# alibaba/pairec

Measured on AMD Instinct MI355X. Metric: ranked items/sec, 5k-cand DNN rank (recall top-5000 of 100M x 128 -> DNN3 -> fuse -> sort), higher is better.
Workload: dtype bf16x3; 1 GPU; configs[1]+[2]: recall 5k of 100000000x128 fp32 table in HBM -> 3-layer DNN rank (256-512-256-1, bf16 MFMA with split hi + lo operands = bf16x3, fp32-accurate scores) -> RankScore fusion (fp64) -> ItemRankScore sort; candidates_per_request=5000, table_rows=100000000, dim=128, table_dist=uniform, batches_in_flight=2, contexts=2, all_batches_on_predicted_thresholds=True, batches_re_run_after_a_failed_plan=0, parallelism=1 GPU

## Files before the change

### pairec_amd/csrc/recall.hip

```cpp
#include "common.hpp"
#include "bitonic_reg.hpp"
#include "split_sort.hpp"

#include <type_traits>

namespace pg {

typedef float f32x16 __attribute__((ext_vector_type(16)));
typedef float f32x4 __attribute__((ext_vector_type(4)));

constexpr int kPieceRows = 32;
constexpr int kPieceCols = 32;
constexpr int kPieceBytes = kPieceRows * kPieceCols * 4;
constexpr int kPieceDmas = kPieceBytes / 1024;
constexpr int kPieceQuads = kPieceCols / 4;
constexpr int kRingSlots = 4;
constexpr int kScanWaves = 8;
constexpr int kScanLdsRing = kScanWaves * kRingSlots * kPieceBytes;
constexpr int kStageCap = 280;
constexpr int kStageBytes = kStageCap * 12 + 512;
constexpr int kScanLds = kScanLdsRing + kScanWaves * kStageBytes;

__device__ __forceinline__ uint32_t f32_ordered_bits(float f) {
    const uint32_t b = __float_as_uint(f);
// ... 260 lines not shown
                    __builtin_amdgcn_s_waitcnt(0x0F70);
                } else {
#pragma unroll
                    for (int r = 0; r < 16; ++r) {
                        const bool p = (pass >> r) & 1u;
                        const uint64_t m = __builtin_amdgcn_ballot_w64(p);
                        if (m != 0) {
                            if (p) {
                                const uint32_t pos = st_n + __builtin_amdgcn_mbcnt_hi((uint32_t)(m >> 32),
                                                         __builtin_amdgcn_mbcnt_lo((uint32_t)m, 0u));
                                const uint32_t row = row0 + (r & 3) + 8 * (r >> 2) + 4 * h;
                                st_key[pos] = topk_key(acc[c][r], row);
                                st_q[pos] = qid;
                            }
                            st_n += __popcll(m);
                        }
                    }
                }
            }
        }
    }
    flush();
    wait_vmcnt<0>();
}

typedef __bf16 bf16x8 __attribute__((ext_vector_type(8)));
typedef float f32x8 __attribute__((ext_vector_type(8)));

constexpr int kScreenMaxNQB = 8;
constexpr int kScreenLds = 163840;
constexpr float kScreenEps = 0.008f;

struct ScreenArgs {
    const void* tab16;
    const uint4* qb16;
    const float* thr_screen;
    uint32_t* susp_cnt;
    uint32_t* susp;
    uint32_t* overflow;
    uint32_t cap, nq, rb_begin, rb_end, row_end, stride, perm_mul, perm_mod;
    const float* blk_norm2;
    const float* eps_unit;
    char* rec;
    uint32_t* rec_cnt;
    uint32_t rec_cap;
    char* rec_pool;
    uint32_t rec_pool_cap, rec_waves;
    uint32_t early_share;
    const float* blk_nxmin;
    const float* l2_b;
    const float* nx_rows;
};

constexpr uint32_t kRecBytes = 80;
constexpr uint32_t kRecOvfWord = 1 + kMaxQueries + 1;

template <int DIM, int NQB, int WAVES, int SPLIT = 1, int VAR = 0, bool I8 = false, int QH = 1, int L2 = 0>
__global__ __launch_bounds__(64 * WAVES, WAVES / 4) void screen_kernel(ScreenArgs a) {
    static_assert(SPLIT == 1 && VAR == 0);
    static_assert(!L2 || (I8 && QH == 1), "squared-Euclidean screen: the int8 kernels of <= 128 queries");
    extern __shared__ __attribute__((aligned(16))) char smem[];
    constexpr int EB = I8 ? 1 : 2;
    constexpr int kCols16 = 128 / EB;
    static_assert(DIM % kCols16 == 0, "a shadow row is a whole number of 128-B lines");
    constexpr int PPB = DIM / kCols16;
    constexpr int NS = kScanLdsRing / (WAVES * kPieceBytes);
    constexpr int ND = kPieceDmas;
    constexpr int KS = DIM * EB / 32;
    typedef int i32x16 __attribute__((ext_vector_type(16)));
    typedef int i32x4 __attribute__((ext_vector_type(4)));
    using AccT = typename std::conditional<I8, i32x16, f32x16>::type;
    using ThrT = typename std::conditional<I8, int, float>::type;
    constexpr int kBLds = QH > 1 ? 2048 : 0;
    constexpr int kStageBytesW = (kScreenLds - kScanLdsRing - kBLds) / WAVES;
    constexpr int NQT = NQB * QH;
    static_assert(QH == 1 || PPB == 1, "query halves: one piece per block");
    constexpr int kCap = (kStageBytesW - NQT * 256 - 16) / 8;
    constexpr int kScanWaves = WAVES;
    const int lane = threadIdx.x & 63;
    const int wave = __builtin_amdgcn_readfirstlane(threadIdx.x >> 6);
    const uint32_t gw = blockIdx.x * kScanWaves + wave;
    const uint32_t W = gridDim.x * kScanWaves;
    const int i32 = lane & 31;
    const int h = lane >> 5;

    uint4 bfrag[NQT][KS];
    ThrT thr_s[NQT];
    float eu[NQT];
    float la[NQT];
    bool active[NQT];
    char* const b_lds = smem + kScreenLds - kBLds;
    if constexpr (QH > 1) {
        if (wave == 0) {
            *reinterpret_cast<uint4*>(b_lds + lane * 16) = a.qb16[((NQT - 1) * KS + KS - 2) * 64 + lane];
            *reinterpret_cast<uint4*>(b_lds + 1024 + lane * 16) = a.qb16[((NQT - 1) * KS + KS - 1) * 64 + lane];
        }
        __syncthreads();
    }
#pragma unroll
    for (int c = 0; c < NQT; ++c) {
#pragma unroll
        for (int ks = 0; ks < KS; ++ks) {
            if (QH > 1 && c == NQT - 1 && ks >= KS - 2) bfrag[c][ks] = make_uint4(0, 0, 0, 0);
            else bfrag[c][ks] = a.qb16[(c * KS + ks) * 64 + lane];
        }
        active[c] = (uint32_t)(c * 32 + i32) < a.nq;
        if constexpr (I8) thr_s[c] = active[c] ? __float_as_int(a.thr_screen[c * 32 + i32]) : 0x7fffffff;
        else thr_s[c] = active[c] ? a.thr_screen[c * 32 + i32] : __builtin_inff();
        eu[c] = (!I8 && active[c]) ? a.eps_unit[c * 32 + i32] : 0.0f;
        if constexpr (L2 != 0) {
            la[c] = active[c] ? a.thr_screen[c * 32 + i32] : __builtin_inff();
            eu[c] = active[c] ? a.l2_b[c * 32 + i32] : 0.0f;
        }
    }
#pragma unroll
    for (int c = 0; c < NQT; ++c) {
#pragma unroll
        for (int ks = 0; ks < KS; ++ks) {
            if (QH > 1 && c == NQT - 1 && ks >= KS - 2) continue;
            if (NQT > 4)
                asm volatile("" : "+a"(bfrag[c][ks].x), "+a"(bfrag[c][ks].y), "+a"(bfrag[c][ks].z), "+a"(bfrag[c][ks].w));
            else
                asm volatile("" : "+v"(bfrag[c][ks].x), "+v"(bfrag[c][ks].y), "+v"(bfrag[c][ks].z), "+v"(bfrag[c][ks].w));
        }
        asm volatile("" : "+v"(thr_s[c]));
        if (!I8 || L2) asm volatile("" : "+v"(eu[c]));
        if (L2) asm volatile("" : "+v"(la[c]));
    }

    uint32_t voff[ND];
#pragma unroll
    for (int n = 0; n < ND; ++n) {
        const int S = n * 64 + lane;
        const int i = S >> 3, p = S & 7;
        voff[n] = (uint32_t)(i * DIM * EB + 16 * ((p + (i >> 1)) & 7));
    }
    const uint32_t lds_wave_u = __builtin_amdgcn_readfirstlane(
        (uint32_t)(uintptr_t)((__attribute__((address_space(3))) char*)smem) + wave * (NS * kPieceBytes));
    char* const lds_ptr = smem + wave * (NS * kPieceBytes);
    const int rd_row = i32 * 128;
    const int rd_rot = (i32 >> 1) * 16;

    const uint32_t total = a.rb_end - a.rb_begin;
    uint32_t first, nblk;
    if (WAVES == 8 && a.early_share != 512) {
        const uint32_t P = gridDim.x * 4;
        const uint32_t pb = (total + P - 1) / P;
        const uint32_t pbase = (blockIdx.x * 4 + (wave & 3)) * pb;
        const uint32_t pend = pbase + pb < total ? pbase + pb : total;
        uint32_t cut = pbase + (uint32_t)(((uint64_t)pb * a.early_share + 512) >> 10);
        if (cut > pend) cut = pend;
        first = wave < 4 ? pbase : cut;
        const uint32_t last = wave < 4 ? cut : pend;
        nblk = first < last ? last - first : 0;
    } else {
        const uint32_t bpw = (total + W - 1) / W;
        first = gw * bpw;
        nblk = first < total ? (total - first < bpw ? total - first : bpw) : 0;
    }
    if (nblk == 0) {
        if (QH > 1 && lane == 0) a.rec_cnt[gw] = 0;
        return;
    }

    constexpr int D = (PPB - 1 + NS - 1) / PPB;
    const bool strided = a.stride != 1;
    const uint32_t L0 = a.rb_begin + first;
    uint32_t walk_slot = strided ? (uint32_t)(((uint64_t)L0 * a.perm_mul) % a.perm_mod) : L0;
    uint32_t walk_n = 0;
    auto next_phys = [&]() -> uint32_t {
        const uint32_t ph = strided ? slot_block(walk_slot, a.stride) : walk_slot;
        if (walk_n + 1 < nblk) {
            ++walk_n;
            if (strided) {
                walk_slot += a.perm_mul;
                if (walk_slot >= a.perm_mod) walk_slot -= a.perm_mod;
            } else {
                ++walk_slot;
            }
        }
        return __builtin_amdgcn_readfirstlane(ph);
    };
    uint32_t phys[D + 1];
#pragma unroll
    for (int j = 0; j <= D; ++j) phys[j] = next_phys();
    auto piece_addr = [&](int rel_piece, uint32_t t, const char*& ub, uint32_t& dst) {
        const uint32_t ph = phys[rel_piece / PPB];
        const char* base = (const char*)a.tab16 + (uint64_t)ph * (uint64_t)(kPieceRows * DIM * EB) + (rel_piece % PPB) * 128;
// ... 2 lines not shown
        ub = (const char*)(((uint64_t)hi << 32) | lo);
        dst = lds_wave_u + __builtin_amdgcn_readfirstlane(t % NS) * kPieceBytes;
    };

    uint32_t* const st_row = reinterpret_cast<uint32_t*>(smem + kScanLdsRing + wave * kStageBytesW);
    uint32_t* const st_q = st_row + kCap;
    uint32_t* const st_cnt = st_q + kCap;
    uint32_t* const st_base = st_cnt + NQT * 32;
    uint32_t st_n = 0;
    auto flush = [&]() {
#pragma unroll
        for (int part = 0; part < (NQT + 1) / 2; ++part)
            if (lane + 64 * part < NQT * 32) st_cnt[lane + 64 * part] = 0;
        for (uint32_t e0 = 0; e0 < st_n; e0 += 64) {
            const uint32_t e = e0 + lane;
            if (e < st_n) atomicAdd(&st_cnt[st_q[e]], 1u);
        }
#pragma unroll
        for (int part = 0; part < (NQT + 1) / 2; ++part) {
            const int q = lane + 64 * part;
            if (q < NQT * 32) {
                const uint32_t c = st_cnt[q];
                st_base[q] = c ? atomicAdd(&a.susp_cnt[q], c) : 0u;
                st_cnt[q] = 0;
            }
        }
        for (uint32_t e0 = 0; e0 < st_n; e0 += 64) {
            const uint32_t e = e0 + lane;
            if (e < st_n) {
                const uint32_t q = st_q[e];
                const uint32_t pos = st_base[q] + atomicAdd(&st_cnt[q], 1u);
                if (pos < a.cap) a.susp[(uint64_t)q * a.cap + pos] = st_row[e];
                else *a.overflow = 1u;
            }
        }
        st_n = 0;
        __builtin_amdgcn_s_waitcnt(0x0F70);
    };

#pragma unroll
    for (int t = 0; t < NS - 1; ++t) {
        const char* src;
        uint32_t dst;
        piece_addr(t, t, src, dst);
#pragma unroll
        for (int n = 0; n < ND; ++n) dma_one(src, dst + n * 1024, voff[n], 0.0f);
    }

    if constexpr (QH > 1) {
        constexpr uint32_t kRecStage = (uint32_t)kStageBytesW / kRecBytes;
        char* const rec_lds = smem + kScanLdsRing + wave * kStageBytesW;
        char* const rec_glb = a.rec + (size_t)gw * a.rec_cap * kRecBytes;
        uint32_t rec_st = 0, rec_total = 0;
        auto rec_flush = [&]() {
            if (rec_total + rec_st > a.rec_cap) {
                uint32_t g = 0;
                if (lane == 0) g = atomicAdd(&a.rec_cnt[a.rec_waves], rec_st);
                g = __builtin_amdgcn_readfirstlane(g);
                if (g + rec_st > a.rec_pool_cap) {
                    if (lane == 0) { *a.overflow = 1u; a.overflow[kRecOvfWord] = 1u; }
                } else {
                    char* const dst = a.rec_pool + (size_t)g * kRecBytes;
                    for (uint32_t o = lane * 16; o < rec_st * kRecBytes; o += 1024)
                        *reinterpret_cast<i32x4*>(dst + o) = *reinterpret_cast<const i32x4*>(rec_lds + o);
                }
            } else {
                char* const dst = rec_glb + (size_t)rec_total * kRecBytes;
                for (uint32_t o = lane * 16; o < rec_st * kRecBytes; o += 1024)
                    *reinterpret_cast<i32x4*>(dst + o) = *reinterpret_cast<const i32x4*>(rec_lds + o);
                rec_total += rec_st;
            }
            rec_st = 0;
        };
        for (uint32_t b = 0; b < nblk; ++b) {
            wait_vmcnt<ND * (NS - 2)>();
            const char* nb_src;
            uint32_t nb_dst;
            piece_addr(NS - 1, b + NS - 1, nb_src, nb_dst);
            const char* slot = lds_ptr + (b % NS) * kPieceBytes + rd_row;
            f32x4 q4[4];
#pragma unroll
            for (int j = 0; j < 4; ++j) q4[j] = *reinterpret_cast<const f32x4*>(slot + (((2 * j + h) * 16 - rd_rot) & 112));
            __builtin_amdgcn_sched_barrier(0);
#pragma unroll
            for (int n = 0; n < ND; ++n)
                dma_one(nb_src, nb_dst + n * 1024, voff[n], q4[n].x);
            const uint32_t cur_phys = phys[0];
#pragma unroll
            for (int j = 0; j < D; ++j) phys[j] = phys[j + 1];
            phys[D] = next_phys();
            const uint32_t row0 = cur_phys * kPieceRows;
#pragma unroll
            for (int half = 0; half < QH; ++half) {
                AccT acc[NQB];
#pragma unroll
                for (int c = 0; c < NQB; ++c)
#pragma unroll
                    for (int r = 0; r < 16; ++r) acc[c][r] = 0;
#pragma unroll
                for (int ksl = 0; ksl < 4; ++ksl)
#pragma unroll
                    for (int c = 0; c < NQB; ++c) {
                        uint4 bq;
                        if (half * NQB + c == NQT - 1 && ksl >= KS - 2) bq = *reinterpret_cast<const uint4*>(b_lds + (ksl - (KS - 2)) * 1024 + lane * 16);
                        else bq = bfrag[half * NQB + c][ksl];
                        acc[c] = __builtin_amdgcn_mfma_i32_32x32x32_i8(__builtin_bit_cast(i32x4, q4[ksl]),
                                                                       __builtin_bit_cast(i32x4, bq), acc[c], 0, 0, 0);
                    }
                uint64_t cmask[NQB];
                bool hit[NQB];
                uint64_t any_mask = 0;
#pragma unroll
                for (int c = 0; c < NQB; ++c) {
                    int m = acc[c][0];
#pragma unroll
                    for (int r = 1; r < 16; ++r) m = acc[c][r] > m ? acc[c][r] : m;
                    hit[c] = m >= thr_s[half * NQB + c];
                    cmask[c] = __builtin_amdgcn_ballot_w64(hit[c]);
                    any_mask |= cmask[c];
                }
                if (any_mask != 0) {
#pragma unroll
                    for (int c = 0; c < NQB; ++c) {
                        if (cmask[c] == 0) continue;
                        uint64_t pend = cmask[c];
                        bool mine = hit[c];
                        for (;;) {
                            const uint32_t n = (uint32_t)__popcll(pend);
                            if (rec_st + n > kRecStage && rec_st != 0) rec_flush();
                            const uint32_t pre = __builtin_amdgcn_mbcnt_hi((uint32_t)(pend >> 32),
                                                                           __builtin_amdgcn_mbcnt_lo((uint32_t)pend, 0u));
                            const bool take = mine && pre < kRecStage;
                            if (take) {
                                char* const r = rec_lds + (rec_st + pre) * kRecBytes;
#pragma unroll
                                for (int jj = 0; jj < 4; ++jj) {
                                    const i32x4 v = {acc[c][4 * jj], acc[c][4 * jj + 1], acc[c][4 * jj + 2], acc[c][4 * jj + 3]};
                                    *reinterpret_cast<i32x4*>(r + 16 * jj) = v;
                                }
                                *reinterpret_cast<uint2*>(r + 64) = make_uint2(row0, (uint32_t)((half * NQB + c) * 32 + i32) | ((uint32_t)h << 8));
                            }
                            rec_st += n < kRecStage ? n : kRecStage;
                            if (n <= kRecStage) break;
                            mine = mine && !take;
                            pend = __builtin_amdgcn_ballot_w64(mine);
                        }
                    }
                }
            }
        }
        rec_flush();
        if (lane == 0) a.rec_cnt[gw] = rec_total;
    } else {
    for (uint32_t b = 0; b < nblk; ++b) {
        AccT acc[NQB];
#pragma unroll
        for (int c = 0; c < NQB; ++c)
#pragma unroll
            for (int r = 0; r < 16; ++r) acc[c][r] = 0;
#pragma unroll
        for (int pc = 0; pc < PPB; ++pc) {
            const uint32_t t = b * PPB + pc;
            wait_vmcnt<ND * (NS - 2)>();
            const char* nb_src;
            uint32_t nb_dst;
            piece_addr(pc + NS - 1, t + NS - 1, nb_src, nb_dst);
            const char* slot = lds_ptr + (t % NS) * kPieceBytes + rd_row;
            f32x4 q4[4];
#pragma unroll
            for (int j = 0; j < 4; ++j) {
                const int quad = 2 * j + h;
                q4[j] = *reinterpret_cast<const f32x4*>(slot + ((quad * 16 - rd_rot) & 112));
            }
            __builtin_amdgcn_sched_barrier(0);
#pragma unroll
            for (int n = 0; n < ND; ++n)
                dma_one(nb_src, nb_dst + n * 1024, voff[n], q4[n].x);
#pragma unroll
            for (int ksl = 0; ksl < 4; ++ksl) {
                const bf16x8 af = __builtin_bit_cast(bf16x8, q4[ksl]);
                const int ks = pc * 4 + ksl;
#pragma unroll
                for (int c = 0; c < NQB; ++c) {
                    if constexpr (I8)
                        acc[c] = __builtin_amdgcn_mfma_i32_32x32x32_i8(__builtin_bit_cast(i32x4, q4[ksl]),
                                                                       __builtin_bit_cast(i32x4, bfrag[c][ks]), acc[c], 0, 0, 0);
                    else
                        acc[c] = __builtin_amdgcn_mfma_f32_32x32x16_bf16(af, __builtin_bit_cast(bf16x8, bfrag[c][ks]), acc[c], 0, 0, 0);
                }
            }
        }
        const uint32_t cur_phys = phys[0];
#pragma unroll
// ... 53 lines not shown
            any_mask |= cmask[c];
        }
        if (any_mask != 0) {
            const uint32_t row0 = cur_phys * kPieceRows;
#pragma unroll
            for (int c = 0; c < NQB; ++c) {
                if (cmask[c] == 0) continue;
                uint32_t m16 = 0;
#pragma unroll
                for (int r = 0; r < 16; ++r) {
                    if constexpr (L2 == 2) {
                        const float g = __fmaf_rn((float)acc[c][r], eu[c], -nxr[r]);
                        asm volatile("v_cmp_nlt_f32 vcc, %1, %2\n\tv_addc_co_u32 %0, vcc, %0, %0, vcc"
                                     : "+v"(m16) : "v"(g), "v"(la[c]) : "vcc");
                    } else if constexpr (I8)
                        asm volatile("v_cmp_ge_i32 vcc, %1, %2\n\tv_addc_co_u32 %0, vcc, %0, %0, vcc"
                                     : "+v"(m16) : "v"(acc[c][r]), "v"(cut[c]) : "vcc");
                    else
                        asm volatile("v_cmp_nlt_f32 vcc, %1, %2\n\tv_addc_co_u32 %0, vcc, %0, %0, vcc"
                                     : "+v"(m16) : "v"(acc[c][r]), "v"(cut[c]) : "vcc");
                }
                if (row0 + kPieceRows > a.row_end) {
#pragma unroll
                    for (int r = 0; r < 16; ++r)
                        if (row0 + (r & 3) + 8 * (r >> 2) + 4 * h >= a.row_end) m16 &= ~(1u << (15 - r));
                }
                for (;;) {
                    const bool p = m16 != 0;
                    const uint64_t bm = __builtin_amdgcn_ballot_w64(p);
                    if (bm == 0) break;
                    const uint32_t n = __popcll(bm);
                    if (st_n + n > (uint32_t)kCap) flush();
                    if (p) {
                        const int r = 15 - __builtin_ctz(m16);
                        const uint32_t pos = st_n + __builtin_amdgcn_mbcnt_hi((uint32_t)(bm >> 32),
                                                 __builtin_amdgcn_mbcnt_lo((uint32_t)bm, 0u));
                        st_row[pos] = row0 + (r & 3) + 8 * (r >> 2) + 4 * h;
                        st_q[pos] = (uint32_t)(c * 32 + i32);
                        m16 &= m16 - 1;
                    }
                    st_n += n;
                }
            }
        }
    }
    }
    if constexpr (QH == 1) flush();
    wait_vmcnt<0>();
}

__device__ __forceinline__ uint32_t rec_mask(const char* r, const float* __restrict__ thr_screen, uint32_t row_end, uint32_t& q,
                                             uint32_t& row0h) {
    typedef int i32x4 __attribute__((ext_vector_type(4)));
    const uint2 tag = *reinterpret_cast<const uint2*>(r + 64);
    q = tag.y & 255u;
    const uint32_t h = (tag.y >> 8) & 1u;
    row0h = tag.x + 4 * h;
    const int t = __float_as_int(thr_screen[q]);
    uint32_t m = 0;
#pragma unroll
    for (int jj = 0; jj < 4; ++jj) {
        const i32x4 v = *reinterpret_cast<const i32x4*>(r + 16 * jj);
#pragma unroll
        for (int e = 0; e < 4; ++e) {
            const int rr = 4 * jj + e;
            if (v[e] >= t && row0h + (rr & 3) + 8 * (rr >> 2) < row_end) m |= 1u << rr;
        }
    }
    return m;
}
constexpr uint32_t kRecPoolSlice = 8192;
__global__ __launch_bounds__(1024) void screen_decode_kernel(const char* __restrict__ rec, const uint32_t* __restrict__ rec_cnt,
                                                             uint32_t rec_cap, uint32_t rec_waves, const char* __restrict__ rec_pool,
                                                             uint32_t rec_pool_cap, const float* __restrict__ thr_screen, uint32_t row_end,
                                                             uint32_t* __restrict__ susp_cnt, uint32_t* __restrict__ susp,
                                                             uint32_t cap, uint32_t* __restrict__ overflow) {
    __shared__ uint32_t cntq[kMaxQueries], baseq[kMaxQueries], nreg[8];
    constexpr uint32_t kKeep = 12288;
    __shared__ uint2 keep[kKeep];
    const bool pool = blockIdx.x >= rec_waves / 8;
    if (threadIdx.x < kMaxQueries) cntq[threadIdx.x] = 0;
    if (threadIdx.x < 8) {
        uint32_t n;
        if (pool) {
            const uint32_t filled = rec_cnt[rec_waves] < rec_pool_cap ? rec_cnt[rec_waves] : rec_pool_cap;
            const uint32_t begin = (blockIdx.x - rec_waves / 8) * kRecPoolSlice;
            n = threadIdx.x == 0 && begin < filled ? (filled - begin < kRecPoolSlice ? filled - begin : kRecPoolSlice) : 0u;
        } else {
            const uint32_t n_raw = rec_cnt[blockIdx.x * 8 + threadIdx.x];
            n = n_raw < rec_cap ? n_raw : rec_cap;
        }
        nreg[threadIdx.x] = n;
    }
    __syncthreads();
    for (int pass = 0; pass < 2; ++pass) {
        uint32_t off = 0;
        for (uint32_t w = 0; w < 8; ++w) {
            const uint32_t n = nreg[w];
            const char* const base = pool ? rec_pool + (size_t)(blockIdx.x - rec_waves / 8) * kRecPoolSlice * kRecBytes
                                          : rec + (size_t)(blockIdx.x * 8 + w) * rec_cap * kRecBytes;
            for (uint32_t e = threadIdx.x; e < n; e += 1024) {
                uint32_t q, row0h, m;
                const uint32_t slot = off + e;
                if (pass == 1 && slot < kKeep) {
                    const uint2 kp = keep[slot];
                    row0h = kp.x;
                    q = kp.y & 0xffffu;
                    m = kp.y >> 16;
                } else {
                    m = rec_mask(base + (size_t)e * kRecBytes, thr_screen, row_end, q, row0h);
                    if (pass == 0 && slot < kKeep) keep[slot] = make_uint2(row0h, q | (m << 16));
                }
                if (m == 0) continue;
                const uint32_t nh = __popc(m);
                if (pass == 0) {
                    atomicAdd(&cntq[q], nh);
                } else {
                    uint32_t pos = baseq[q] + atomicAdd(&cntq[q], nh);
                    if (pos + nh > cap) { *overflow = 1u; continue; }
                    while (m) {
                        const uint32_t rr = __builtin_ctz(m);
                        m &= m - 1;
                        susp[(uint64_t)q * cap + pos++] = row0h + (rr & 3) + 8 * (rr >> 2);
                    }
                }
            }
            off += n;
        }
        __syncthreads();
        if (pass == 0 && threadIdx.x < kMaxQueries) {
            const uint32_t c = cntq[threadIdx.x];
            baseq[threadIdx.x] = c ? atomicAdd(&susp_cnt[threadIdx.x], c) : 0u;
            cntq[threadIdx.x] = 0;
        }
        __syncthreads();
    }
}

template <int DIM>
__device__ __forceinline__ void rescore_gather(f32x4 (&buf)[16], const float* __restrict__ tab, uint32_t row, int ph, int lane) {
#pragma unroll
    for (int i = 0; i < 16; ++i) {
        const uint32_t r_i = (uint32_t)__shfl((int)row, 4 * i + (lane >> 4), 64);
        buf[i] = reinterpret_cast<const f32x4*>(tab + (size_t)r_i * DIM + ph * 64)[lane & 15];
    }
}
template <int ROWB>
__device__ __forceinline__ void rescore_walk(const f32x4 (&buf)[16], char* my, const float* qs, int ph, int lane, float& s) {
#pragma unroll
    for (int i = 0; i < 16; ++i)
        *reinterpret_cast<f32x4*>(my + (4 * i + (lane >> 4)) * ROWB + (lane & 15) * 16) = buf[i];
    __builtin_amdgcn_fence(__ATOMIC_RELEASE, "wavefront");
    __builtin_amdgcn_wave_barrier();
#pragma unroll
    for (int k = 0; k < 16; ++k) {
        const float4 x = *reinterpret_cast<const float4*>(my + lane * ROWB + k * 16);
        const float4 y = *reinterpret_cast<const float4*>(&qs[ph * 64 + 4 * k]);
        s = __fmaf_rn(x.x, y.x, s);
        s = __fmaf_rn(x.y, y.y, s);
        s = __fmaf_rn(x.z, y.z, s);
        s = __fmaf_rn(x.w, y.w, s);
        if ((k & 3) == 3) __builtin_amdgcn_sched_barrier(0);
    }
    __builtin_amdgcn_wave_barrier();
}

template <int DIM, bool L2 = false>
__global__ __launch_bounds__(256) void rescore_kernel(const float* __restrict__ tab, const float* __restrict__ qpad,
                                                      const float* __restrict__ thr,
                                                      const uint32_t* __restrict__ susp,
                                                      const uint32_t* __restrict__ susp_cnt, uint32_t cap,
                                                      uint32_t* __restrict__ cnt, uint64_t* __restrict__ cand,
                                                      uint32_t* __restrict__ overflow, uint32_t scap, uint32_t n_rows,
                                                      const float* __restrict__ nx = nullptr, const float* __restrict__ nqv = nullptr,
                                                      RowFilter filter = RowFilter()) {
    constexpr int kRowB = 64 * 4 + 16;
// ... 69 lines not shown
        uint32_t pos = base_s + before;
        for (int j = 0; j < w; ++j) pos += wsum[j];
        if (keep) {
            if (pos < cap) cand[(uint64_t)q * cap + pos] = topk_key(s, row);
            else *overflow = 1u;
        }
        __syncthreads();
        row = row_next;
    }
    if (n_raw > scap && threadIdx.x == 0) *overflow = 1u;
}

__global__ void screen_prep_kernel(const float* __restrict__ qpad, uint32_t dim,
                                   uint4* __restrict__ qb16, float* __restrict__ eps) {
    const uint32_t KS = dim / 16;
    const uint32_t i = blockIdx.x * blockDim.x + threadIdx.x;
    if (i < (uint32_t)kScreenMaxNQB * KS * 64) {
        const uint32_t lane = i & 63, ks = (i >> 6) % KS, c = (i >> 6) / KS;
        const float* q = qpad + (size_t)(c * 32 + (lane & 31)) * dim + ks * 16 + 8 * (lane >> 5);
        uint32_t w[4];
        for (int e = 0; e < 4; ++e) {
            auto rne = [](float x) -> uint32_t {
                uint32_t b = __float_as_uint(x);
                if ((b & 0x7FFFFFFFu) > 0x7F800000u) return (b >> 16) | 0x40u;
                b += 0x7FFFu + ((b >> 16) & 1u);
                return b >> 16;
            };
            w[e] = rne(q[2 * e]) | (rne(q[2 * e + 1]) << 16);
        }
        qb16[i] = make_uint4(w[0], w[1], w[2], w[3]);
    }
    if (i < (uint32_t)kMaxQueries) {
        double ss = 0.0;
        for (uint32_t k = 0; k < dim; ++k) {
            const double v = (double)qpad[(size_t)i * dim + k];
            ss += v * v;
        }
        eps[i] = (float)(sqrt(ss) * (double)kScreenEps * 1.0001) + 1e-30f;
    }
}

__global__ void screen_thr_kernel(const float* __restrict__ thr, const float* __restrict__ eps, float max_norm,
                                  float* __restrict__ thr_screen) {
    const uint32_t q = threadIdx.x;
    if (q >= (uint32_t)kMaxQueries) return;
    const float t = thr[q], e = eps[q];
    float v = t;
    if (!(e == e) || e > 1e28f || !(t == t) || !(e * max_norm < 1e35f)) v = -__builtin_inff();
    thr_screen[q] = v;
}

__global__ __launch_bounds__(128) void screen_prep8_kernel(const float* __restrict__ qpad, uint32_t dim,
                                                            float max_norm, float resid, uint4* __restrict__ qb8,
                                                            float* __restrict__ eps, float* __restrict__ qscale) {
    __shared__ float sq[32];
    const uint32_t tid = threadIdx.x, c = blockIdx.x;
    {
        const uint32_t ql = tid >> 2, qi = c * 32 + ql, part = tid & 3, per = dim / 4;
        const float* q = qpad + (size_t)qi * dim + part * per;
        float mx = 0.0f;
        bool bad = false;
        for (uint32_t k = 0; k < per; ++k) {
            const float v = fabsf(q[k]);
            if (!(v <= 3.0e38f)) bad = true;
            mx = fmaxf(mx, v);
        }
        mx = fmaxf(mx, __shfl_xor(mx, 1, 64));
        mx = fmaxf(mx, __shfl_xor(mx, 2, 64));
        bad = (__shfl_xor((int)bad, 1, 64) | (int)bad) != 0;
        bad = (__shfl_xor((int)bad, 2, 64) | (int)bad) != 0;
        const float sc = fmaxf(mx / 127.0f, 1e-30f);
        double ss = 0.0, dd = 0.0;
        for (uint32_t k = 0; k < per; ++k) {
            const double v = (double)q[k];
            int Q = __float2int_rn(q[k] / sc);
            Q = Q > 127 ? 127 : (Q < -127 ? -127 : Q);
            const double d = v - (double)sc * (double)Q;
            ss += v * v;
            dd += d * d;
        }
        ss += __shfl_xor(ss, 1, 64);
        ss += __shfl_xor(ss, 2, 64);
        dd += __shfl_xor(dd, 1, 64);
        dd += __shfl_xor(dd, 2, 64);
        if (part == 0) {
            const double nq = sqrt(ss), dq = sqrt(dd);
            const double e = ((double)resid * nq + ((double)max_norm + (double)resid) * dq) * 1.0001 +
                             1e-5 * (double)max_norm * nq + 1e-30;
            eps[qi] = bad ? __builtin_nanf("") : (float)(e * 1.000001);
            qscale[qi] = sc;
            sq[ql] = sc;
        }
    }
    __syncthreads();
    const uint32_t KS = dim / 32;
    for (uint32_t i = tid; i < KS * 64; i += blockDim.x) {
        const uint32_t lane = i & 63, ks = i >> 6;
        const uint32_t ql = lane & 31;
        const float* q = qpad + (size_t)(c * 32 + ql) * dim + ks * 32 + 16 * (lane >> 5);
        const float sc = sq[ql];
        uint32_t w[4];
        for (int e = 0; e < 4; ++e) {
            uint32_t word = 0;
            for (int b = 0; b < 4; ++b) {
                int Q = __float2int_rn(q[4 * e + b] / sc);
                Q = Q > 127 ? 127 : (Q < -127 ? -127 : Q);
                word |= (uint32_t)(Q & 0xff) << (8 * b);
            }
            w[e] = word;
        }
        qb8[(c * KS + ks) * 64 + lane] = make_uint4(w[0], w[1], w[2], w[3]);
    }
}

__global__ void screen_thr8_kernel(const float* __restrict__ thr, const float* __restrict__ eps,
                                   const float* __restrict__ qscale, float s_x, float* __restrict__ thr_screen) {
    const uint32_t q = threadIdx.x;
    if (q >= (uint32_t)kMaxQueries) return;
    const float t = thr[q], e = eps[q];
    int T = (int)0x80000000;
    if (e == e && e <= 1e30f && t == t && t > -__builtin_inff()) {
        const double v = floor(((double)t - (double)e) / ((double)s_x * (double)qscale[q])) - 1.0;
        T = v >= 2147483647.0 ? 0x7fffffff : (v <= -2147483648.0 ? (int)0x80000000 : (int)v);
    }
    thr_screen[q] = __int_as_float(T);
}

__global__ void screen_thr8_l2_kernel(const float* __restrict__ thr, const float* __restrict__ eps, const float* __restrict__ qscale,
                                      const float* __restrict__ nqv, float s_x, float max_norm, float* __restrict__ a_out,
                                      float* __restrict__ b_out, int per_row) {
    const uint32_t q = threadIdx.x;
    if (q >= (uint32_t)kMaxQueries) return;
    const float t = thr[q], e = eps[q];
    const double nq = (double)nqv[q], N = (double)max_norm;
    const double sq = (double)s_x * (double)qscale[q];
    float A = -__builtin_inff(), B = 0.0f;
    if (e == e && e <= 1e30f && t == t && t > -__builtin_inff() && sq > 0.0 && nq == nq && nq < 1e30) {
        const double delta = 2e-6 * (N * N + nq + 2.0 * N * sqrt(nq)) + 1e-30;
        if (per_row) {
            const double c = (double)t - 2.0 * delta + nq - 2.0 * (double)e;
            A = (float)(c - fabs(c) * 1e-6 - 1e-30);
            B = (float)(2.0 * sq);
            if (!(A == A) || !(B == B) || B > 1e30f) { A = -__builtin_inff(); B = 0.0f; }
        } else {
            const double a = (((double)t - delta + nq) * 0.5 - (double)e) / sq;
            const double b = 0.5 / sq;
            A = (float)(a - fabs(a) * 1e-6 - 1.0);
            B = (float)(b * (1.0 - 1e-6));
            if (!(A == A) || !(B == B) || B > 1e30f) { A = -__builtin_inff(); B = 0.0f; }
        }
    }
    a_out[q] = A;
    b_out[q] = B;
}
__global__ void block_nxmin_kernel(const float* __restrict__ nx, uint64_t rows, float* __restrict__ out, uint32_t nblocks,
                                   double* __restrict__ stats) {
    const uint32_t b = blockIdx.x * blockDim.x + threadIdx.x;
    double slack = 0.0, sum = 0.0;
    if (b < nblocks) {
        float m = __builtin_inff();
        for (uint32_t i = 0; i < (uint32_t)kPieceRows; ++i) {
            const uint64_t r = (uint64_t)b * kPieceRows + i;
            if (r < rows) m = fminf(m, nx[r]);
        }
// ... 1282 lines not shown
    bool last_was_i4m = false;
    bool last_was_r2 = false;
    bool exact_chunks = false;

    explicit PlanRun(RecallJob* job) : j(job), ctx(job->ctx), t(job->t), rs(job->rs) {}

    int scan_range(uint32_t rb, uint32_t cb, uint32_t st, bool thr_is_open, bool allow_i4 = false) {
        std::vector<hipEvent_t>& pool = *j->events;
        while (pool.size() < 2 * (size_t)(n_ev + 1)) {
            hipEvent_t e;
            PG_HIP(hipEventCreate(&e));
            pool.push_back(e);
        }
        if (j->timers) PG_HIP(hipEventRecord(pool[2 * n_ev], ctx->stream));
        const uint32_t nq = j->nq;
        if (j->screen && !thr_is_open && !exact_chunks) {
            ScreenArgs sa;
            sa.tab16 = t->shadow_is_i8 ? (const void*)t->d8 : (const void*)t->d16;
            sa.blk_norm2 = t->dnorm2;
            sa.eps_unit = rs.eps;
            sa.qb16 = rs.qb16;
            sa.thr_screen = rs.thr_screen;
            sa.susp_cnt = rs.susp_cnt;
            sa.susp = rs.susp;
            sa.overflow = rs.overflow;
            sa.cap = rs.cap;
            sa.nq = nq;
            sa.rb_begin = rb;
            sa.rb_end = rb + cb;
            sa.row_end = j->rows;
            sa.stride = st;
            sa.perm_mul = j->perm_mul;
            sa.perm_mod = j->sample_blocks;
            int rc2;
            const bool records = t->shadow_is_i8 && nq > 128;
            sa.rec = nullptr;
            sa.rec_cnt = nullptr;
            sa.rec_cap = 0;
            sa.rec_pool = nullptr;
            sa.rec_pool_cap = sa.rec_waves = 0;
            sa.early_share = records ? ctx->knobs.screen_early_share : ctx->knobs.screen_early_share_narrow;
            sa.blk_nxmin = j->l2 && !j->l2_per_row ? t->d_nxmin : nullptr;
            sa.nx_rows = j->l2 && j->l2_per_row ? t->d_nx : nullptr;
            sa.l2_b = j->l2 ? rs.thr_ref : nullptr;
            const uint32_t rec_waves = (uint32_t)ctx->num_cus * 8u;
            if (records) {
                const uint64_t rsc = t->rec_scale ? t->rec_scale : 1;
                uint32_t cap_w = (uint32_t)(((uint64_t)kMaxQueries * j->k * 4 * rsc / rec_waves + 255) / 256 * 256);
                const uint32_t pairs = (uint32_t)ctx->num_cus * 4u;
                const uint32_t pb = (kCandSlack / 2 / kPieceRows + pairs - 1) / pairs;
                const uint32_t es = sa.early_share > 512 ? sa.early_share : 1024 - sa.early_share;
                uint32_t eb = (uint32_t)(((uint64_t)pb * es + 512) >> 10) + 1;
                if (eb > pb) eb = pb;
                const uint32_t floor_w = eb * 512;
                if (cap_w < floor_w) cap_w = floor_w;
                const uint32_t pool_cap = (uint32_t)(((uint64_t)kMaxQueries * j->k * 2 * rsc + kRecPoolSlice - 1) / kRecPoolSlice * kRecPoolSlice);
                if ((rc2 = scratch_carve(ctx, kSlotHitRecords, [&](Carve& c) {
                        sa.rec_cnt = c.take<uint32_t>((size_t)rec_waves + 1);
                        sa.rec = (char*)c.bytes(((size_t)rec_waves * cap_w + pool_cap) * kRecBytes);
                    }))) return rc2;
                sa.rec_cap = cap_w;
                sa.rec_pool = sa.rec + (size_t)rec_waves * cap_w * kRecBytes;
                sa.rec_pool_cap = pool_cap;
                sa.rec_waves = rec_waves;
                PG_HIP(hipMemsetAsync(sa.rec_cnt, 0, (size_t)(rec_waves + 1) * 4, ctx->stream));
            }
            if (!susp_clean) PG_HIP(hipMemsetAsync(rs.susp_cnt, 0, sizeof(uint32_t) * kMaxQueries, ctx->stream));
            susp_clean = false;
            last_full_screened = true;
            last_was_r2 = false;
            const bool i4 = j->screen4 && allow_i4 && st == 1 && (rb & 1) == 0 && (((rb + cb) & 1) == 0 || rb + cb == j->nblocks);
            const bool i4m = j->screen4m && allow_i4 && st == 1 && (rb & 1) == 0 && (((rb + cb) & 1) == 0 || rb + cb == j->nblocks);
            const uint32_t scap = i4 ? rs.cap * (uint32_t)(kMaxQueries / kI4MaxQueries) : rs.cap;
            const uint64_t r_begin = (uint64_t)rb * kPieceRows;
            const uint64_t r_end = (uint64_t)(rb + cb) * kPieceRows < j->rows ? (uint64_t)(rb + cb) * kPieceRows : j->rows;
            if (i4) {
                if ((rc2 = screen4_launch(ctx, t, rs, nq, (uint32_t)r_begin, (uint32_t)r_end, scap, j->l2 ? rs.pred_ms : nullptr))) return rc2;
                j->scan_bytes += (r_end - r_begin) * (j->l2 ? 72 : 68);
            } else if (i4m) {
                if ((rc2 = screen4m_launch(ctx, t, rs, nq, (uint32_t)r_begin, (uint32_t)r_end, rs.cap * (uint32_t)(kMaxQueries / kI4mMaxQueries), susp2_clean))) return rc2;
                susp2_clean = false;
                j->scan_bytes += (r_end - r_begin) * 68;
                last_was_i4m = true;
            } else {
                last_was_i4m = false;
                if ((rc2 = dispatch_screen(ctx, t->dim, t->shadow_is_i8, sa))) return rc2;
                if (records) {
                    screen_decode_kernel<<<rec_waves / 8 + sa.rec_pool_cap / kRecPoolSlice, 1024, 0, ctx->stream>>>(
                        sa.rec, sa.rec_cnt, sa.rec_cap, rec_waves, sa.rec_pool, sa.rec_pool_cap, rs.thr_screen, j->rows,
                                                                            rs.susp_cnt, rs.susp, rs.cap, rs.overflow);
                    PG_HIP(hipGetLastError());
                }
                j->scan_bytes += (uint64_t)cb * kPieceRows * t->dim * (t->shadow_is_i8 ? 1 : 2);
            }
            j->scanned_rows += (uint64_t)cb * kPieceRows;
            const dim3 rg(i4 ? screen4_rescore_blocks() : kRescoreBlocksPerQuery, nq);
            const bool r2 = j->stage2 && t->shadow_is_i8 && !i4 && !i4m && !j->l2 && t->dim == 128;
            if (r2) {
                if ((rc2 = rescreen16_launch(ctx, t, rs, nq))) return rc2;
                last_was_r2 = true;
                rescore_kernel<128><<<rg, 256, 0, ctx->stream>>>(t->d, rs.qpad, rs.thr, rs.susp2, rs.susp2w_cnt, rs.cap,
                                                                 rs.cnt, rs.cand[cur], rs.overflow, rs.cap, j->rows, nullptr, nullptr, j->filter);
            } else if (j->l2)
                rescore_kernel<128, true><<<rg, 256, 0, ctx->stream>>>(t->d, rs.qpad, rs.thr, rs.susp, rs.susp_cnt, rs.cap, rs.cnt,
                                                                       rs.cand[cur], rs.overflow, scap, j->rows, t->d_nx, rs.pred_ms, j->filter);
            else if (t->dim == 64)
                rescore_kernel<64><<<rg, 256, 0, ctx->stream>>>(t->d, rs.qpad, rs.thr, rs.susp, rs.susp_cnt, rs.cap,
// ... 61 lines not shown
    }
    int grow_scan(uint32_t nb, uint32_t st, uint32_t kk, double growth, bool safe) {
        uint32_t rb = 0;
        while (rb < nb) {
            uint32_t chunk_rows;
            if (rb == 0) {
                chunk_rows = next_pow2(8 * kk);
                if (chunk_rows < 2048) chunk_rows = 2048;
                if (chunk_rows > kFirstChunkRows || chunk_rows < kk) chunk_rows = kFirstChunkRows;
            } else {
                const uint64_t grow = (uint64_t)((double)rb * kPieceRows * (growth - 1.0));
                chunk_rows = grow > 0xFFFFFFE0ull ? 0xFFFFFFE0u : (uint32_t)grow;
            }
            if (safe && chunk_rows > kCandSlack / 2) chunk_rows = kCandSlack / 2;
            uint32_t cb = chunk_rows / kPieceRows;
            if (cb > nb - rb) cb = nb - rb;
            int rc2;
            if ((rc2 = scan_range(rb, cb, st, rb == 0))) return rc2;
            rb += cb;
            if ((rc2 = refresh(kk))) return rc2;
        }
        return PG_OK;
    }
};
}

int recall_job_enqueue(RecallJob* j) {
    pg_ctx* ctx = j->ctx;
    const pg_table* t = j->t;
    const Knobs& kn = ctx->knobs;
    if (j->next_plan >= j->n_plans) {
        set_error("recall: candidate overflow in safe mode (internal error)");
        return PG_ERR_DEVICE;
    }
    const int plan = j->plans[j->next_plan];
    int rc;
    if ((rc = recall_scratch(ctx, t->dim, j->k, &j->rs))) return rc;
    j->d_count = j->rs.overflow + 1;
    if (plan == kIndexPlan) return index_plan_enqueue(j, kStatusCopyWords);
    PlanRun r(j);
    RecallScratch& rs = j->rs;
    recall_init_kernel<<<(kMaxQueries * t->dim + 255) / 256, 256, 0, ctx->stream>>>(
        j->d_queries, j->nq, t->dim, rs.qpad, rs.thr, rs.cnt, rs.overflow);
    PG_HIP(hipGetLastError());
    if (j->l2) {
        query_norm2_kernel<<<1, kMaxQueries, 0, ctx->stream>>>(rs.qpad, t->dim, rs.pred_ms);
        PG_HIP(hipGetLastError());
    }
    r.no_i8 = plan == kPredict && j->screen4;
    if (j->screen) {
        if (!r.no_i8) {
            if (t->shadow_is_i8)
                screen_prep8_kernel<<<j->nq <= 32 ? 1u : (j->nq <= 64 ? 2u : (j->nq <= 128 ? 4u : 8u)), 128, 0, ctx->stream>>>(
                    rs.qpad, t->dim, t->max_norm, t->resid8, rs.qb16, rs.eps, rs.qscale);
            else
                screen_prep_kernel<<<(kScreenMaxNQB * (t->dim / 16) * 64 + 255) / 256, 256, 0, ctx->stream>>>(
                    rs.qpad, t->dim, rs.qb16, rs.eps);
            PG_HIP(hipGetLastError());
        }
        if (j->screen4 && (rc = screen4_prep_launch(ctx, t, rs))) return rc;
        if (j->screen4m) {
            if ((rc = screen4m_prep_launch(ctx, rs, j->nq))) return rc;
            r.susp2_clean = true;
        }
        if (j->stage2 && (rc = rescreen16_prep_launch(ctx, t, rs, j->nq))) return rc;
    }
    const bool observe = j->pred_observe && (plan == kPilot || plan == kPredict);
    if (observe || plan == kPredict) {
        pred_query_kernel<<<j->nq, 128, 0, ctx->stream>>>(rs.qpad, t->d_pred, rs.pred_ms, plan == kPredict ? rs.thr : nullptr,
                                                          (float)j->z_lo);
        PG_HIP(hipGetLastError());
    }
    while (j->events->size() < 2) {
        hipEvent_t e;
        PG_HIP(hipEventCreate(&e));
        j->events->push_back(e);
    }
    bool refined = false;
    r.n_ev = 1;
    j->timers = !ctx->timers_off;
    if (j->timers) PG_HIP(hipEventRecord((*j->events)[0], ctx->stream));
    if (plan == kPredict && !r.no_i8) {
        screen_thr8_kernel<<<1, kMaxQueries, 0, ctx->stream>>>(rs.thr, rs.eps, rs.qscale, t->s8, rs.thr_screen);
        PG_HIP(hipGetLastError());
    }
    if (plan == kPilot || plan == kPredict) {
      if (plan == kPilot) {
        const uint32_t seed_rows = kn.seed_rows;
        const uint64_t sample_rows = (uint64_t)j->sample_blocks * kPieceRows;
        if (j->screen && kn.pilot_growth <= 0.0 && sample_rows > 8ull * seed_rows && j->k_pilot < seed_rows / 4) {
            const double mu = (double)seed_rows * (double)j->k_pilot / (double)sample_rows;
            uint32_t m0 = 1;
            for (double term = exp(-mu), cdf = term; 1.0 - cdf > 1e-9 && m0 < seed_rows; ++m0) {
                term *= mu / (double)m0;
                cdf += term;
            }
            ++m0;
            const uint32_t sb = seed_rows / kPieceRows;
            if ((rc = r.scan_range(0, sb, j->stride, true))) return rc;
            if ((rc = r.refresh(m0))) return rc;
            if ((rc = r.scan_range(sb, j->sample_blocks - sb, j->stride, false))) return rc;
            if ((rc = r.refresh(j->k_pilot))) return rc;
        } else {
            if ((rc = r.grow_scan(j->sample_blocks, j->stride, j->k_pilot, kn.pilot_growth > 0.0 ? kn.pilot_growth : 8.0, false))) return rc;
        }
      }
        if (plan == kPilot) PG_HIP(hipMemsetAsync(rs.cnt, 0, sizeof(uint32_t) * kMaxQueries, ctx->stream));
// ... 759 lines not shown
```

Before: 265.5 million ranked items/s.

## Switch query-half int8 screen to 16x16x64 MFMA with compact hit records

```diff
diff --git a/pairec_amd/csrc/recall.hip b/pairec_amd/csrc/recall.hip
--- a/pairec_amd/csrc/recall.hip
+++ b/pairec_amd/csrc/recall.hip
@@ -336,7 +336,7 @@
     const float* nx_rows;
 };
 
-constexpr uint32_t kRecBytes = 80;
+constexpr uint32_t kRecBytes = 48;
 constexpr uint32_t kRecOvfWord = 1 + kMaxQueries + 1;
 
 template <int DIM, int NQB, int WAVES, int SPLIT = 1, int VAR = 0, bool I8 = false, int QH = 1, int L2 = 0>
@@ -355,7 +355,7 @@
     typedef int i32x4 __attribute__((ext_vector_type(4)));
     using AccT = typename std::conditional<I8, i32x16, f32x16>::type;
     using ThrT = typename std::conditional<I8, int, float>::type;
-    constexpr int kBLds = QH > 1 ? 2048 : 0;
+    constexpr int kBLds = QH > 1 ? 3072 : 0;
     constexpr int kStageBytesW = (kScreenLds - kScanLdsRing - kBLds) / WAVES;
     constexpr int NQT = NQB * QH;
     static_assert(QH == 1 || PPB == 1, "query halves: one piece per block");
@@ -374,11 +374,14 @@
     float la[NQT];
     bool active[NQT];
     char* const b_lds = smem + kScreenLds - kBLds;
+    int* const thr_lds = reinterpret_cast<int*>(b_lds + 2048);
     if constexpr (QH > 1) {
         if (wave == 0) {
             *reinterpret_cast<uint4*>(b_lds + lane * 16) = a.qb16[((NQT - 1) * KS + KS - 2) * 64 + lane];
             *reinterpret_cast<uint4*>(b_lds + 1024 + lane * 16) = a.qb16[((NQT - 1) * KS + KS - 1) * 64 + lane];
         }
+        if (threadIdx.x < (uint32_t)kMaxQueries)
+            thr_lds[threadIdx.x] = threadIdx.x < a.nq ? __float_as_int(a.thr_screen[threadIdx.x]) : 0x7fffffff;
         __syncthreads();
     }
 #pragma unroll
@@ -389,7 +392,8 @@
             else bfrag[c][ks] = a.qb16[(c * KS + ks) * 64 + lane];
         }
         active[c] = (uint32_t)(c * 32 + i32) < a.nq;
-        if constexpr (I8) thr_s[c] = active[c] ? __float_as_int(a.thr_screen[c * 32 + i32]) : 0x7fffffff;
+        if constexpr (QH > 1) thr_s[c] = 0;
+        else if constexpr (I8) thr_s[c] = active[c] ? __float_as_int(a.thr_screen[c * 32 + i32]) : 0x7fffffff;
         else thr_s[c] = active[c] ? a.thr_screen[c * 32 + i32] : __builtin_inff();
         eu[c] = (!I8 && active[c]) ? a.eps_unit[c * 32 + i32] : 0.0f;
         if constexpr (L2 != 0) {
@@ -407,7 +411,7 @@
             else
                 asm volatile("" : "+v"(bfrag[c][ks].x), "+v"(bfrag[c][ks].y), "+v"(bfrag[c][ks].z), "+v"(bfrag[c][ks].w));
         }
-        asm volatile("" : "+v"(thr_s[c]));
+        if (QH == 1) asm volatile("" : "+v"(thr_s[c]));
         if (!I8 || L2) asm volatile("" : "+v"(eu[c]));
         if (L2) asm volatile("" : "+v"(la[c]));
     }
@@ -417,7 +421,7 @@
     for (int n = 0; n < ND; ++n) {
         const int S = n * 64 + lane;
         const int i = S >> 3, p = S & 7;
-        voff[n] = (uint32_t)(i * DIM * EB + 16 * ((p + (i >> 1)) & 7));
+        voff[n] = (uint32_t)(i * DIM * EB + 16 * ((p + (QH > 1 ? (i & 6) : (i >> 1))) & 7));
     }
     const uint32_t lds_wave_u = __builtin_amdgcn_readfirstlane(
         (uint32_t)(uintptr_t)((__attribute__((address_space(3))) char*)smem) + wave * (NS * kPieceBytes));
@@ -526,6 +530,9 @@
         char* const rec_lds = smem + kScanLdsRing + wave * kStageBytesW;
         char* const rec_glb = a.rec + (size_t)gw * a.rec_cap * kRecBytes;
         uint32_t rec_st = 0, rec_total = 0;
+        const int r16 = lane & 15, g16 = lane >> 4;
+        const int rot16 = (r16 & 6) * 16;
+        const uint32_t tag16 = (uint32_t)r16 | ((uint32_t)g16 << 8);
         auto rec_flush = [&]() {
             if (rec_total + rec_st > a.rec_cap) {
                 uint32_t g = 0;
@@ -551,10 +558,11 @@
             const char* nb_src;
             uint32_t nb_dst;
             piece_addr(NS - 1, b + NS - 1, nb_src, nb_dst);
-            const char* slot = lds_ptr + (b % NS) * kPieceBytes + rd_row;
+            const char* slot = lds_ptr + (b % NS) * kPieceBytes + r16 * 128;
             f32x4 q4[4];
 #pragma unroll
-            for (int j = 0; j < 4; ++j) q4[j] = *reinterpret_cast<const f32x4*>(slot + (((2 * j + h) * 16 - rd_rot) & 112));
+            for (int j = 0; j < 4; ++j)
+                q4[j] = *reinterpret_cast<const f32x4*>(slot + (((4 * (j & 1) + g16) * 16 - rot16) & 112) + 2048 * (j >> 1));
             __builtin_amdgcn_sched_barrier(0);
 #pragma unroll
             for (int n = 0; n < ND; ++n)
@@ -566,36 +574,43 @@
             const uint32_t row0 = cur_phys * kPieceRows;
 #pragma unroll
             for (int half = 0; half < QH; ++half) {
-                AccT acc[NQB];
-#pragma unroll
-                for (int c = 0; c < NQB; ++c)
-#pragma unroll
-                    for (int r = 0; r < 16; ++r) acc[c][r] = 0;
-#pragma unroll
-                for (int ksl = 0; ksl < 4; ++ksl)
-#pragma unroll
-                    for (int c = 0; c < NQB; ++c) {
-                        uint4 bq;
-                        if (half * NQB + c == NQT - 1 && ksl >= KS - 2) bq = *reinterpret_cast<const uint4*>(b_lds + (ksl - (KS - 2)) * 1024 + lane * 16);
-                        else bq = bfrag[half * NQB + c][ksl];
-                        acc[c] = __builtin_amdgcn_mfma_i32_32x32x32_i8(__builtin_bit_cast(i32x4, q4[ksl]),
-                                                                       __builtin_bit_cast(i32x4, bq), acc[c], 0, 0, 0);
-                    }
-                uint64_t cmask[NQB];
-                bool hit[NQB];
+                constexpr int NC = 2 * NQB;
+                i32x4 acc[2][NC];
+                int thr16[NC];
+#pragma unroll
+                for (int c = 0; c < NC; ++c) thr16[c] = thr_lds[(half * NC + c) * 16 + r16];
+#pragma unroll
+                for (int ks = 0; ks < 2; ++ks) {
+#pragma unroll
+                    for (int c = 0; c < NC; ++c)
+#pragma unroll
+                        for (int rh = 0; rh < 2; ++rh) {
+                            constexpr int kLdsFrag = NQT * KS - 2;
+                            const int f = (half * NC + c) * 2 + ks;
+                            uint4 bq;
+                            if (f >= kLdsFrag) bq = *reinterpret_cast<const uint4*>(b_lds + (f - kLdsFrag) * 1024 + lane * 16);
+                            else bq = bfrag[f / KS][f % KS];
+                            const i32x4 c0 = ks == 0 ? i32x4{0, 0, 0, 0} : acc[rh][c];
+                            acc[rh][c] = __builtin_amdgcn_mfma_i32_16x16x64_i8(__builtin_bit_cast(i32x4, q4[2 * rh + ks]),
+                                                                               __builtin_bit_cast(i32x4, bq), c0, 0, 0, 0);
+                        }
+                    if (ks == 0) __builtin_amdgcn_sched_barrier(0);
+                }
+                uint64_t cmask[NC];
+                bool hit[NC];
                 uint64_t any_mask = 0;
 #pragma unroll
-                for (int c = 0; c < NQB; ++c) {
-                    int m = acc[c][0];
-#pragma unroll
-                    for (int r = 1; r < 16; ++r) m = acc[c][r] > m ? acc[c][r] : m;
-                    hit[c] = m >= thr_s[half * NQB + c];
+                for (int c = 0; c < NC; ++c) {
+                    int m = acc[0][c][0];
+#pragma unroll
+                    for (int r = 1; r < 8; ++r) m = acc[r >> 2][c][r & 3] > m ? acc[r >> 2][c][r & 3] : m;
+                    hit[c] = m >= thr16[c];
                     cmask[c] = __builtin_amdgcn_ballot_w64(hit[c]);
                     any_mask |= cmask[c];
                 }
                 if (any_mask != 0) {
 #pragma unroll
-                    for (int c = 0; c < NQB; ++c) {
+                    for (int c = 0; c < NC; ++c) {
                         if (cmask[c] == 0) continue;
                         uint64_t pend = cmask[c];
                         bool mine = hit[c];
@@ -607,12 +622,11 @@
                             const bool take = mine && pre < kRecStage;
                             if (take) {
                                 char* const r = rec_lds + (rec_st + pre) * kRecBytes;
-#pragma unroll
-                                for (int jj = 0; jj < 4; ++jj) {
-                                    const i32x4 v = {acc[c][4 * jj], acc[c][4 * jj + 1], acc[c][4 * jj + 2], acc[c][4 * jj + 3]};
-                                    *reinterpret_cast<i32x4*>(r + 16 * jj) = v;
-                                }
-                                *reinterpret_cast<uint2*>(r + 64) = make_uint2(row0, (uint32_t)((half * NQB + c) * 32 + i32) | ((uint32_t)h << 8));
+                                *reinterpret_cast<i32x4*>(r) = acc[0][c];
+                                *reinterpret_cast<i32x4*>(r + 16) = acc[1][c];
+                                uint32_t tag = tag16;
+                                asm volatile("" : "+v"(tag));
+                                *reinterpret_cast<uint2*>(r + 32) = make_uint2(row0, tag + (uint32_t)((half * NC + c) * 16));
                             }
                             rec_st += n < kRecStage ? n : kRecStage;
                             if (n <= kRecStage) break;
@@ -772,19 +786,19 @@
 __device__ __forceinline__ uint32_t rec_mask(const char* r, const float* __restrict__ thr_screen, uint32_t row_end, uint32_t& q,
                                              uint32_t& row0h) {
     typedef int i32x4 __attribute__((ext_vector_type(4)));
-    const uint2 tag = *reinterpret_cast<const uint2*>(r + 64);
+    const uint2 tag = *reinterpret_cast<const uint2*>(r + 32);
     q = tag.y & 255u;
-    const uint32_t h = (tag.y >> 8) & 1u;
-    row0h = tag.x + 4 * h;
+    const uint32_t g = (tag.y >> 8) & 3u;
+    row0h = tag.x + 4 * g;
     const int t = __float_as_int(thr_screen[q]);
     uint32_t m = 0;
 #pragma unroll
-    for (int jj = 0; jj < 4; ++jj) {
+    for (int jj = 0; jj < 2; ++jj) {
         const i32x4 v = *reinterpret_cast<const i32x4*>(r + 16 * jj);
 #pragma unroll
         for (int e = 0; e < 4; ++e) {
             const int rr = 4 * jj + e;
-            if (v[e] >= t && row0h + (rr & 3) + 8 * (rr >> 2) < row_end) m |= 1u << rr;
+            if (v[e] >= t && row0h + (rr & 3) + 16 * (rr >> 2) < row_end) m |= 1u << rr;
         }
     }
     return m;
@@ -841,7 +855,7 @@
                     while (m) {
                         const uint32_t rr = __builtin_ctz(m);
                         m &= m - 1;
-                        susp[(uint64_t)q * cap + pos++] = row0h + (rr & 3) + 8 * (rr >> 2);
+                        susp[(uint64_t)q * cap + pos++] = row0h + (rr & 3) + 16 * (rr >> 2);
                     }
                 }
             }
@@ -1017,7 +1031,7 @@
 
 __global__ __launch_bounds__(128) void screen_prep8_kernel(const float* __restrict__ qpad, uint32_t dim,
                                                             float max_norm, float resid, uint4* __restrict__ qb8,
-                                                            float* __restrict__ eps, float* __restrict__ qscale) {
+                                                            float* __restrict__ eps, float* __restrict__ qscale, uint32_t wide) {
     __shared__ float sq[32];
     const uint32_t tid = threadIdx.x, c = blockIdx.x;
     {
@@ -1060,9 +1074,9 @@
     __syncthreads();
     const uint32_t KS = dim / 32;
     for (uint32_t i = tid; i < KS * 64; i += blockDim.x) {
-        const uint32_t lane = i & 63, ks = i >> 6;
-        const uint32_t ql = lane & 31;
-        const float* q = qpad + (size_t)(c * 32 + ql) * dim + ks * 32 + 16 * (lane >> 5);
+        const uint32_t lane = i & 63, ks = wide ? (i >> 6) & 1 : i >> 6;
+        const uint32_t ql = wide ? 16 * (i >> 7) + (lane & 15) : lane & 31;
+        const float* q = qpad + (size_t)(c * 32 + ql) * dim + (wide ? ks * 64 + 16 * (lane >> 4) : ks * 32 + 16 * (lane >> 5));
         const float sc = sq[ql];
         uint32_t w[4];
         for (int e = 0; e < 4; ++e) {
@@ -1074,7 +1088,7 @@
             }
             w[e] = word;
         }
-        qb8[(c * KS + ks) * 64 + lane] = make_uint4(w[0], w[1], w[2], w[3]);
+        qb8[c * KS * 64 + i] = make_uint4(w[0], w[1], w[2], w[3]);
     }
 }
 
@@ -2463,7 +2477,7 @@
                 const uint32_t es = sa.early_share > 512 ? sa.early_share : 1024 - sa.early_share;
                 uint32_t eb = (uint32_t)(((uint64_t)pb * es + 512) >> 10) + 1;
                 if (eb > pb) eb = pb;
-                const uint32_t floor_w = eb * 512;
+                const uint32_t floor_w = eb * 1024;
                 if (cap_w < floor_w) cap_w = floor_w;
                 const uint32_t pool_cap = (uint32_t)(((uint64_t)kMaxQueries * j->k * 2 * rsc + kRecPoolSlice - 1) / kRecPoolSlice * kRecPoolSlice);
                 if ((rc2 = scratch_carve(ctx, kSlotHitRecords, [&](Carve& c) {
@@ -2631,7 +2645,8 @@
         if (!r.no_i8) {
             if (t->shadow_is_i8)
                 screen_prep8_kernel<<<j->nq <= 32 ? 1u : (j->nq <= 64 ? 2u : (j->nq <= 128 ? 4u : 8u)), 128, 0, ctx->stream>>>(
-                    rs.qpad, t->dim, t->max_norm, t->resid8, rs.qb16, rs.eps, rs.qscale);
+                    rs.qpad, t->dim, t->max_norm, t->resid8, rs.qb16, rs.eps, rs.qscale,
+                    j->nq > 128 && !j->l2 ? 1u : 0u);
             else
                 screen_prep_kernel<<<(kScreenMaxNQB * (t->dim / 16) * 64 + 255) / 256, 256, 0, ctx->stream>>>(
                     rs.qpad, t->dim, rs.qb16, rs.eps);
```

Measured after the change: 280.7 million ranked items/s (median of 6 runs). 5.7% higher.
